# microsoft/DCVC

Hardware: AMD Instinct MI355X
Metric: 1080p YUV420 intra encode+decode pictures per second (DCVC-UF-Intra (DMCI), real rANS bit streams, q_index in {0,16,32,48,63}; sequential loop: compress then decompress per picture) (higher is better)
Workload: dtype f16

## Files before the change

### dcvc_amd/csrc/capi_ops.hip

```cpp
#include "capi_common.h"
#include <initializer_list>
#include <memory>
#include <mutex>
#include <stdexcept>
#include "dcvc_amd_ops.h"
#include "kernels/ops.h"
#include "rans/code_length.h"

namespace {

using dcvc::half_t;

inline const half_t* H(const void* p) { return static_cast<const half_t*>(p); }
inline half_t* H(void* p) { return static_cast<half_t*>(p); }
inline hipStream_t S(void* s) { return static_cast<hipStream_t>(s); }

const half_t* zero_page()
{
    static half_t* z = nullptr;
    static std::once_flag once;
    std::call_once(once, [] {
        dcvc::hip_check(hipMalloc(&z, 4096), "hipMalloc(zero page)");
        dcvc::hip_check(hipMemset(z, 0, 4096), "hipMemset(zero page)");
    });
// ... 321 lines not shown
        d.b3 = H(b3); d.b0 = H(b0); d.b2 = H(b2); d.q = H(q); d.q2 = H(q2);
        d.y = H(y); d.ldy = ldy;
        d.pixels = pixels; d.c = c; d.ci = ci; d.shortcut = shortcut != 0;
        d.wfin = wf.half(); d.bfin = H(bfin); d.qfin = H(qfin); d.yfin = H(yfin); d.ldyfin = ldyfin; d.nfin = nfin;
        dcvc::dcb_nsplit(d, st);
    });
}

int dcvc_dcb_nsplit_dw_supported(int c, int ci, int pixels)
{
    return dcvc::dcb_nsplit_dw_supported(c, ci, pixels) ? 1 : 0;
}

int dcvc_dcb_nsplit_dw(const void* t1, int ldt, const void* wdw, int width, const void* x, int ldx, const void* w3, const void* b3,
                       const void* w0, const void* b0, const void* w2, const void* b2, const void* q, const void* q2,
                       const void* w1n, const void* b1n, void* t1n, int ldt1,
                       const void* wfin, const void* bfin, const void* qfin, void* yfin, int ldyfin, int nfin,
                       void* y, int ldy, int pixels, int c, int ci, int shortcut, void* stream)
{
    return dcvc::guarded([&] {
        dcvc::kernels_init();
        nsplit_check_shape(c, ci);
        if (!t1 || !wdw || !w3 || !w0 || !w2) throw std::invalid_argument("dcb_nsplit_dw: missing operand");
        if (!dcvc::dcb_nsplit_dw_supported(c, ci, pixels)) throw std::invalid_argument("dcb_nsplit_dw: no kernel variant with the depthwise conv inside for this block shape");
        if (wfin != nullptr && !dcvc::dcb_nsplit_fin_supported(c, ci, nfin)) throw std::invalid_argument("dcb_nsplit_dw: no kernel variant for this closing conv");
        if (static_cast<long long>(pixels) * ldt * 2 >= (1LL << 31)) throw std::invalid_argument("dcb_nsplit_dw: dc.0's output must span less than 2 GiB (32-bit byte offsets inside the launch)");
        hipStream_t st = S(stream);
        const AsyncBuf wmain(dcvc::dcb_nsplit_main_halves(c, ci) * 2, st);
        dcvc::dcb_nsplit_pack_main(H(w3), H(w0), H(w2), c, ci, wmain.half(), st);
        std::unique_ptr<AsyncBuf> wnext, wf;
        if (w1n != nullptr) {
            wnext = std::make_unique<AsyncBuf>(dcvc::dcb_nsplit_dc0_halves(c, ci) * 2, st);
            dcvc::dcb_nsplit_pack_dc0(H(w1n), c, ci, wnext->half(), st);
        }
        if (wfin != nullptr) {
            wf = std::make_unique<AsyncBuf>(dcvc::dcb_nsplit_fin_halves(c, nfin) * 2, st);
            dcvc::dcb_nsplit_pack_fin(H(wfin), c, nfin, wf->half(), st);
        }
        dcvc::DcbNsplitDesc d;
        d.t1 = H(t1); d.ldt = ldt; d.wdw = H(wdw); d.width = width; d.x = H(x); d.ldx = ldx;
        d.wmain = wmain.half();
        d.wnext = wnext ? wnext->half() : nullptr;
        d.b3 = H(b3); d.b0 = H(b0); d.b2 = H(b2); d.b1n = H(b1n); d.q = H(q); d.q2 = H(q2);
        d.t1n = H(t1n); d.ldt1 = ldt1; d.y = H(y); d.ldy = ldy;
        d.pixels = pixels; d.c = c; d.ci = ci; d.shortcut = shortcut != 0;
        if (wf) { d.wfin = wf->half(); d.bfin = H(bfin); d.qfin = H(qfin); d.yfin = H(yfin); d.ldyfin = ldyfin; d.nfin = nfin; }
        dcvc::dcb_nsplit(d, st);
// ... 443 lines not shown
```

### dcvc_amd/csrc/kernels/dcb_nsplit.hip

```cpp
#include "dcb_nsplit8_kernel.h"

namespace dcvc {

using namespace nsplit;

namespace {

struct Share {
    int hi, lo, act;
    bool by_pair;
    __host__ __device__ explicit Share(int n)
    {
        by_pair = n % 128 == 0;
        if (by_pair) {
            const int q = n / 128;
            hi = (q + 1) / 2; lo = q / 2; act = 4;
        } else {
            const int tn = n / 32;
            hi = (tn + 7) / 8;
            const int rem = tn - 4 * hi;
            lo = rem <= 0 ? 0 : (rem + 3) / 4;
            act = lo == 0 ? 0 : rem / lo;
        }
    }
// ... 84 lines not shown
           (c == 512 && ci == 256) || (c == 256 && ci == 128) ||
           (c == 384 && ci == 192) ||
           (c == 192 && ci == 192);
}

bool dcb_nsplit_fin_supported(int c, int ci, int nn)
{
    static const bool off = [] { const char* e = getenv("DCVC_NSPLIT_FIN"); return e != nullptr && atoi(e) == 0; }();
    if (off || !dcb_nsplit_shape(c, ci)) return false;
    if (c == 256 && ci == 128) return nn == 128 || nn == 192 || nn == 256;
    if (c == 256 && ci == 256) return nn == 192;
    if (c == 512 && ci == 512) return nn == 256 || nn == 512;
    if (c == 768 && ci == 768) return nn == 768;
    if (c == 384 && ci == 192) return nn == 384;
    return false;
}

static bool nsplit_wide(int pixels, int c)
{
    static const bool narrow_all = [] { const char* e = getenv("DCVC_NSPLIT_PX"); return e != nullptr && atoi(e) == 32; }();
    return pixels >= 64 * 200 && c < 768 && !narrow_all;
}

bool dcb_nsplit_dw_supported(int c, int ci, int pixels)
{
    static const bool off = [] { const char* e = getenv("DCVC_NSPLIT_DW"); return e != nullptr && atoi(e) == 0; }();
    if (off || pixels <= 0) return false;
    return (c == 256 && ci == 128) || (c == 384 && ci == 192 && !nsplit_wide(pixels, c));
}

void dcb_nsplit_dw_hook(const half_t* t1, const half_t* wdw, int width)
{
    g_dw_hook_t1 = t1; g_dw_hook_taps = wdw; g_dw_hook_width = width;
}

void dcb_nsplit_timeline_buffer(long long* device_buffer)
{
    g_ns_timeline = device_buffer;
}

size_t dcb_nsplit_main_halves(int c, int ci)
{
    const Share sc(c);
    return (2ull * 4 * (sc.hi + sc.lo) * (ci / 16) + 1ull * (ci / 8) * (c / 16)) * 512;
}
size_t dcb_nsplit_dc0_halves(int c, int ci)
{
    return ci % 128 == 0 ? 1ull * (ci / 32) * (c / 16) * 512 : dcb_nsplit_fin_halves(c, ci);
}

size_t dcb_nsplit_fin_halves(int c, int nn)
// ... 33 lines not shown
}

int dcb_nsplit_waves()
{
    return 8;
}

int dcb_nsplit_mode()
{
    static const int mode = [] { const char* e = getenv("DCVC_NSPLIT"); return e != nullptr ? atoi(e) : 2; }();
    return mode;
}

bool dcb_nsplit_supported(int c, int cdc, int cffn)
{
    static const bool core_off = [] { const char* e = getenv("DCVC_NO_DCB_CORE"); return e != nullptr && atoi(e) != 0; }();
    if (core_off || dcb_nsplit_mode() == 0 || cdc != cffn || !dcb_nsplit_shape(c, cdc)) return false;
    return cdc == c || dcb_nsplit_mode() >= 2;
}

void dcb_nsplit(const DcbNsplitDesc& desc, hipStream_t stream)
{
    DcbNsplitDesc d = desc;
    if (g_dw_hook_t1 != nullptr && d.t1 == nullptr && dcb_nsplit_dw_supported(d.c, d.ci, d.pixels) && d.pixels % g_dw_hook_width == 0) {
        d.t2 = nullptr; d.t1 = g_dw_hook_t1; d.wdw = g_dw_hook_taps; d.width = g_dw_hook_width;
    }
    if (!dcb_nsplit_shape(d.c, d.ci)) {
        throw std::invalid_argument("dcb_nsplit: (block width, inner width) must be (256, 256), (384, 384), (512, 512), (768, 768), (512, 256), (256, 128), (384, 192) or (192, 192)");
    }
    if (d.pixels <= 0) throw std::invalid_argument("dcb_nsplit: empty problem");
    if ((d.ldt % 8) || (d.ldx % 8) || (d.ldy % 8) || (d.wnext && d.ldt1 % 8)) {
        throw std::invalid_argument("dcb_nsplit: leading dimensions must be multiples of 8 channels");
    }
    if (d.t1 != nullptr) {
        if (d.t2 != nullptr) throw std::invalid_argument("dcb_nsplit: either the depthwise conv's output (t2) or its input (t1)");
        if (!dcb_nsplit_dw_supported(d.c, d.ci, d.pixels)) throw std::invalid_argument("dcb_nsplit: no kernel with the depthwise conv inside for this block shape and size");
        if (!d.wdw || d.width <= 0 || d.pixels % d.width != 0) throw std::invalid_argument("dcb_nsplit: depthwise conv inside needs its taps and the picture's width");
        if (d.t1 == d.t1n) throw std::invalid_argument("dcb_nsplit: dc.0's output for the next block must not overwrite this block's (neighbouring workgroups read it)");
    }
    if ((!d.t2 && !d.t1) || !d.x || !d.wmain || !d.b3 || !d.b0 || !d.b2 || (!d.y && !d.wfin) || (d.wnext && (!d.b1n || !d.t1n))) {
        throw std::invalid_argument("dcb_nsplit: missing operand");
    }
    if (d.wfin != nullptr) {
        if (d.wnext != nullptr) throw std::invalid_argument("dcb_nsplit: a block either hands dc.0 to the next block or closes the chain");
        if (!dcb_nsplit_fin_supported(d.c, d.ci, d.nfin)) throw std::invalid_argument("dcb_nsplit: no kernel for this closing conv");
        if (!d.bfin || !d.yfin || d.ldyfin % 8) throw std::invalid_argument("dcb_nsplit: closing conv needs bias, output and a leading dimension in units of 8");
    }
    NsParams p{};
    p.t2 = d.t2; p.ldt = d.ldt; p.x = d.x; p.ldx = d.ldx;
    p.t1 = d.t1; p.wdw = d.wdw; p.W = d.width;
    p.wmain = reinterpret_cast<const half8*>(d.wmain); p.wnext = reinterpret_cast<const half8*>(d.wnext);
    p.b3 = d.b3; p.b0 = d.b0; p.b2 = d.b2; p.b1n = d.b1n; p.q = d.q; p.q2 = d.q2;
    p.wsilu = wsilu_table_device();
    p.y = d.y; p.ldy = d.ldy; p.t1n = d.t1n; p.ldt1 = d.ldt1; p.M = d.pixels; p.shortcut = d.shortcut ? 1 : 0;
    p.timeline = g_ns_timeline;
    if (d.wfin != nullptr) {
        p.wnext = reinterpret_cast<const half8*>(d.wfin); p.b1n = d.bfin; p.qf = d.qfin; p.t1n = d.yfin; p.ldt1 = d.ldyfin;
    }
    const bool wide = nsplit_wide(d.pixels, d.c);
    const int next = d.wfin != nullptr ? d.nfin : d.wnext != nullptr ? 1 : 0;
    if (d.t1 != nullptr && d.c == 384) nsplit8::run_384_192_dw(p, next, stream);
    else if (d.t1 != nullptr) nsplit8::run_256_128_dw(p, wide, next, stream);
    else if (d.c == 192) nsplit8::run_192_192(p, wide, next, stream);
    else if (d.c == 384 && d.ci == 192) nsplit8::run_384_192(p, wide, next, stream);
    else if (d.c == 384) nsplit8::run_384_384(p, wide, next, stream);
    else if (d.c == 768) nsplit8::run_768_768(p, wide, next, stream);
    else if (d.c == 512 && d.ci == 512) nsplit8::run_512_512(p, wide, next, stream);
    else if (d.c == 512) nsplit8::run_512_256(p, wide, next, stream);
    else if (d.ci == 256) nsplit8::run_256_256(p, wide, next, stream);
    else nsplit8::run_256_128(p, wide, next, stream);
}

}
```

### dcvc_amd/csrc/kernels/dcb_nsplit8_kernel.h

```cpp
#pragma once
#include "dcb_nsplit_common.h"

namespace dcvc {
namespace nsplit8 {

using nsplit::align16k;
using nsplit::lds_dma16;
using nsplit::NsParams;
using nsplit::R;
using nsplit::static_for;
using nsplit::TABLE_BYTES;
using nsplit::uint4v;

constexpr int NTHREADS = 512;
#ifndef NS8_RING
#define NS8_RING 8
#endif
constexpr int RING = NS8_RING;
#ifndef NS8_RING1
#define NS8_RING1 8
#endif
#ifndef NS8_AHEAD
#define NS8_AHEAD 2
#endif
#ifndef NS8_AHEAD_WIDE
#define NS8_AHEAD_WIDE 1
#endif
#ifndef NS8_GATHERS
#define NS8_GATHERS 8
#endif
constexpr int GB = NS8_GATHERS;

#ifndef NS8_TRIPLE
#define NS8_TRIPLE 1
#endif
template <int C, int CI, int PXT, int NEXT = 1, int DW = 0>
struct Lay {
    static constexpr int CIP = (CI + 127) / 128 * 128;
    static constexpr int CP = (C + 127) / 128 * 128;
    static constexpr int BUF_A = 32 * PXT * CIP * 2, BUF_B = 32 * PXT * CP * 2;
    static constexpr int NB = NEXT > 1 ? NEXT : CI;
    static constexpr int BIAS_FLOATS = 2 * C + 4 * CI + NB;
    static constexpr int CONSTS = BIAS_FLOATS * 4 + 2 * C * 2;
    static constexpr bool FIT4 = 2 * BUF_A + BUF_B + 4 * TABLE_BYTES + CONSTS <= 160 * 1024 && (2 * BUF_A + BUF_B) % 16384 == 0;
    static constexpr bool FIT1 = 2 * BUF_A + BUF_B + 1 * TABLE_BYTES + CONSTS <= 160 * 1024 && (2 * BUF_A + BUF_B) % 4096 == 0;
    static constexpr bool TRIPLE = NS8_TRIPLE != 0 && (FIT4 || FIT1);
    static constexpr int RT = TRIPLE ? (FIT4 ? 4 : 1) : R;
    static constexpr int OFF_B = BUF_A;
    static constexpr int OFF_A2 = BUF_A + BUF_B;
    static constexpr int OFF_TABLE = TRIPLE ? 2 * BUF_A + BUF_B : align16k(BUF_A + BUF_B);
    static constexpr int OFF_BIAS = OFF_TABLE + RT * TABLE_BYTES;
    static constexpr int OFF_Q = OFF_BIAS + BIAS_FLOATS * 4;
    static constexpr int run_chunks(int nw)
    {
        const int pxw = 32 * PXT / nw, pcs = ((pxw + 2) * (CI / 8) + 63) / 64;
        return (nw - 1) * pxw * (CI / 8) + pcs * 64;
    }
    static constexpr int rows_per_run()
    {
        const int ch = run_chunks(8) > run_chunks(4) ? run_chunks(8) : run_chunks(4);
        const int r = (ch + CI / 8 - 1) / (CI / 8);
        return r > 32 * PXT + 2 ? r : 32 * PXT + 2;
    }
    static constexpr int RH = rows_per_run();
    static constexpr int OFF_WDW = OFF_Q + 2 * C * 2;
    static constexpr int OFF_ZERO = OFF_WDW + 9 * CI * 2;
    static constexpr int OFF_H = (OFF_ZERO + 16 + 1023) & ~1023;
    static constexpr int BYTES = DW != 0 ? OFF_H + 3 * RH * CI * 2 : OFF_Q + 2 * C * 2;
    static_assert(BYTES <= 160 * 1024, "LDS budget");
    static_assert(DW == 0 || TRIPLE, "depthwise conv inside: needs the second t2 buffer");
};

template <int C, int CI>
struct Geo {
    static constexpr int KS_C = C / 16, KS_I = CI / 16;
    static constexpr int QC = C / 128, QI = CI / 128;
    static constexpr int HI_C = (QC + 1) / 2, LO_C = QC / 2;
    static constexpr int HI_I = (QI + 1) / 2, LO_I = QI / 2;
    static constexpr bool I_BY_PAIR = CI % 128 == 0;
    static constexpr int PAIRS = CI / 16, P0_HI = (PAIRS + 7) / 8, P0_LO = (PAIRS - 4 * P0_HI) / 4;
    static constexpr int TP = 2;
    static constexpr int n0(bool hiw) { return 2 * (hiw ? P0_HI : P0_LO); }
    static constexpr int np(bool hiw) { return hiw ? P0_HI : P0_LO; }
    static constexpr bool C_BY_PAIR = C % 128 == 0;
    static constexpr bool EVEN = HI_C == LO_C && HI_I == LO_I && I_BY_PAIR && C_BY_PAIR && P0_HI == P0_LO;
    static constexpr int nt_c(bool hiw) { return C_BY_PAIR ? (hiw ? HI_C : LO_C) : (nt_f(C, hiw) > 0 ? nt_f(C, hiw) : 0); }
    static constexpr int nt_i(bool hiw) { return I_BY_PAIR ? (hiw ? HI_I : LO_I) : nt_f(CI, hiw); }
    static constexpr int f_dc3(bool hiw) { return nt_c(hiw) * KS_I; }
    static constexpr int f_ffn0(bool hiw) { return n0(hiw) * KS_C; }
    static constexpr int f_main(bool hiw) { return 2 * f_dc3(hiw) + f_ffn0(hiw); }
    static constexpr int f_dc0(bool hiw) { return nt_i(hiw) * KS_C; }
// ... 8 lines not shown
    static_assert(C % 64 == 0 && CI % 64 == 0 && 4 * (P0_HI + P0_LO) == PAIRS && P0_LO >= 1, "channel counts the eight waves can share");
};

template <int C, int CI, int PXT, int NEXT, int DW, bool HIW>
__device__ __forceinline__ void block_body(const NsParams& p, char* const smem)
{
    using G = Geo<C, CI>;
    constexpr int RING = PXT == 1 ? NS8_RING1 : NS8_RING;
    constexpr bool FIN = NEXT > 1;
    static_assert(!FIN || G::fin_ok(NEXT), "closing conv: a width the eight waves can share");
    static_assert(G::I_BY_PAIR || G::fin_ok(CI), "dc.0: an inner width the eight waves can share");
    static_assert(G::C_BY_PAIR || G::fin_ok(C), "a block width the eight waves can share");
    constexpr int PX = 32 * PXT;
    constexpr int KS_C = G::KS_C, KS_I = G::KS_I;
    constexpr int NT_C = G::nt_c(HIW), NP = G::np(HIW), TP = G::TP;
    constexpr int F_DC3 = G::f_dc3(HIW), F_FFN0 = G::f_ffn0(HIW), F_MAIN = G::f_main(HIW), F_DC0 = G::f_next(NEXT, HIW);
    constexpr int NT_N = G::nt_next(NEXT, HIW);
    constexpr int CIP = Lay<C, CI, PXT, NEXT, DW>::CIP;
    constexpr int CP = Lay<C, CI, PXT, NEXT, DW>::CP;
    constexpr int CH_C = CP / 8, CH_I = CIP / 8;
    constexpr int PITCH_C = CP * 2, PITCH_I = CIP * 2;
    using L = Lay<C, CI, PXT, NEXT, DW>;
    constexpr bool TRIPLE = L::TRIPLE;
    constexpr int RT = L::RT;
    constexpr int OFF_B = L::OFF_B, OFF_A2 = L::OFF_A2;
    constexpr int OFF_TABLE = L::OFF_TABLE;
    constexpr int OFF_BIAS = L::OFF_BIAS;
    constexpr int BIAS_FLOATS = L::BIAS_FLOATS;
    constexpr int OFF_Q = L::OFF_Q;
    constexpr int TOTAL = F_MAIN + (NEXT ? F_DC0 : 0);
    static_assert((PX * CH_C) % NTHREADS == 0 && (PX * CH_I) % NTHREADS == 0, "tile rows must split evenly over the threads");

    const int tid = threadIdx.x;
    const int lane = tid & 63;
    const int wave = __builtin_amdgcn_readfirstlane(tid >> 6);
    const int simd = wave & 3;
    const int px = lane & 31;
    const int hi = lane >> 5;
    const int ntiles = (p.M + PX - 1) / PX;
    const bool banded = DW != 0 && (gridDim.x & 7) == 0 && ntiles >= static_cast<int>(gridDim.x);
    const int band0 = banded ? static_cast<int>((blockIdx.x & 7) * ntiles) >> 3 : 0;
    const int band_n = banded ? (static_cast<int>(((blockIdx.x & 7) + 1) * ntiles) >> 3) - band0 : 0;
    int slot = blockIdx.x >> 3;
    int tile = banded ? band0 + slot : static_cast<int>(blockIdx.x);
    bool first_tile = true;
    int m0 = tile * PX;
// ... 1 lines not shown
    if ((lds_base & 16383u) != 0) __builtin_trap();
    const bool upper = wave >= 4;
    const int cb_c = G::C_BY_PAIR ? 32 * (simd * G::QC + (upper ? G::HI_C : 0))
                   : HIW ? 32 * wave * G::nf_hi(C) : 32 * (4 * G::nf_hi(C) + (wave - 4) * G::nf_lo(C));
    const bool c_on = G::C_BY_PAIR || HIW || (wave - 4) < G::act_lo(C);
    const int cb_x = c_on ? cb_c : 0;
    const int cb_0 = HIW ? wave * (32 * G::n0(true)) : 4 * 32 * G::n0(true) + (wave - 4) * (32 * G::n0(false));
    constexpr bool BY_PAIR = !FIN && G::I_BY_PAIR;
    constexpr int NN = FIN ? NEXT : CI;
    const int cb_n = BY_PAIR ? 32 * (simd * G::QI + (upper ? G::HI_I : 0))
                   : HIW ? 32 * wave * G::nf_hi(NN) : 32 * (4 * G::nf_hi(NN) + (wave - 4) * G::nf_lo(NN));
    const bool nx_on = BY_PAIR || HIW || (wave - 4) < G::act_lo(NN);
    const long long rt0 = static_cast<long long>(__builtin_amdgcn_s_memrealtime());
    int stamp_no = 0;
    auto stamp = [&]() {
        if (p.timeline != nullptr && tid == 0 && stamp_no < 29 && first_tile) {
            p.timeline[static_cast<size_t>(blockIdx.x) * 32 + stamp_no] = static_cast<long long>(__builtin_readcyclecounter());
        }
        ++stamp_no;
    };
    stamp();

    static_assert(RT == 4 || RT == 1, "table slots per thread, spelled out");
    const float4 tab0 = p.wsilu[min(tid / RT, WSILU_SEGMENTS - 1)], tab1 = p.wsilu[min((tid + NTHREADS) / RT, WSILU_SEGMENTS - 1)];
    constexpr int CONST_UNITS = (BIAS_FLOATS + 2 * C) / 8;
    constexpr int CONST_PER_THREAD = (CONST_UNITS + NTHREADS - 1) / NTHREADS;
    static_assert(CONST_PER_THREAD <= 2, "two named registers below");
    auto const_unit = [&](int k) {
        const int ch = min(tid + k * NTHREADS, CONST_UNITS - 1) * 8;
        const half_t* src = ch < C ? p.b3 + ch
                          : ch < C + 4 * CI ? p.b0 + (ch - C)
                          : ch < 2 * C + 4 * CI ? p.b2 + (ch - C - 4 * CI)
                          : ch < BIAS_FLOATS ? (p.b1n != nullptr ? p.b1n + (ch - 2 * C - 4 * CI) : p.b2)
                          : ch < BIAS_FLOATS + C ? (p.q != nullptr ? p.q + (ch - BIAS_FLOATS) : p.b2)
                          : (p.q2 != nullptr ? p.q2 + (ch - BIAS_FLOATS - C) : p.b2);
        return *reinterpret_cast<const half8*>(src);
    };
    const half8 cv0 = const_unit(0), cv1 = const_unit(CONST_PER_THREAD > 1 ? 1 : 0);
    static_assert(DW == 0 || 9 * CI / 8 <= NTHREADS, "the depthwise taps: one 16-byte unit per thread");
    half8 wdv = {0, 0, 0, 0, 0, 0, 0, 0};
    if constexpr (DW != 0) wdv = *reinterpret_cast<const half8*>(p.wdw + min(tid, 9 * CI / 8 - 1) * 8);
    const float* const lb3 = reinterpret_cast<const float*>(smem + OFF_BIAS);
    const float* const lb0 = lb3 + C;
    const float* const lb2 = lb3 + C + 4 * CI;
    const float* const lb1n = lb3 + 2 * C + 4 * CI;
    const half_t* const lq = reinterpret_cast<const half_t*>(smem + OFF_Q);
    const half_t* const lq2 = lq + C;
    unsigned tab = lds_base + OFF_TABLE + (lane & (RT - 1)) * 16;

    constexpr int FM_HI = G::f_main(true), FM_LO = G::f_main(false), FD_HI = G::f_next(NEXT, true), FD_LO = G::f_next(NEXT, false);
    unsigned wsm = static_cast<unsigned>((HIW ? wave * FM_HI : 4 * FM_HI + (wave - 4) * FM_LO) * 64 + lane) * 16u;
    unsigned wsn = static_cast<unsigned>((HIW ? wave * FD_HI : nx_on ? 4 * FD_HI + (wave - 4) * FD_LO : 0) * 64 + lane) * 16u;
    const __amdgpu_buffer_rsrc_t rs_main = __builtin_amdgcn_make_buffer_rsrc(const_cast<half8*>(p.wmain), 0, 0x7fffffff, 0x00020000);
    const __amdgpu_buffer_rsrc_t rs_next = __builtin_amdgcn_make_buffer_rsrc(const_cast<half8*>(NEXT != 0 ? p.wnext : p.wmain), 0, 0x7fffffff, 0x00020000);
    half8 ring[RING];
    auto issue = [&](auto f_tag) {
        constexpr int f = decltype(f_tag)::value;
        if constexpr (f < F_MAIN) {
            ring[f % RING] = __builtin_bit_cast(half8, __builtin_amdgcn_raw_buffer_load_b128(rs_main, wsm + static_cast<unsigned>(f & 3) * 1024u, (f >> 2) * 4096, 0));
        } else if constexpr (f < TOTAL) {
            constexpr int g = f - F_MAIN;
            ring[f % RING] = __builtin_bit_cast(half8, __builtin_amdgcn_raw_buffer_load_b128(rs_next, wsn + static_cast<unsigned>(g & 3) * 1024u, (g >> 2) * 4096, 0));
        }
    };
// ... 87 lines not shown
        for (int i = 0; i < STEPS; ++i) {
            if (i + 1 < STEPS) taps(i + 1, v[(i + 1) & 1]);
            __builtin_amdgcn_sched_barrier(0);
            const int n = i * 64 + (tidv & 63);
            const int r = wi * PXW + n / CH_H, pc = n % CH_H;
            if constexpr (!FIXED_CHUNK) {
#pragma unroll
                for (int k = 0; k < 9; ++k) wt[k] = *reinterpret_cast<const half8*>(smem + L::OFF_WDW + (k * CI + pc * 8) * 2);
            }
            float acc[8];
#pragma unroll
            for (int e = 0; e < 8; ++e) acc[e] = 0.f;
#pragma unroll
            for (int k = 0; k < 9; ++k)
#pragma unroll
                for (int e = 0; e < 8; ++e) acc[e] = fmaf(static_cast<float>(v[i & 1][k][e]), static_cast<float>(wt[k][e]), acc[e]);
            half8 o;
#pragma unroll
            for (int e = 0; e < 8; ++e) o[e] = to_half(acc[e]);
            if (ITEMS % 64 == 0 || n < ITEMS) *reinterpret_cast<half8*>(smem + dst + r * PITCH_I + ((pc ^ (r & 15)) << 4)) = o;
            __builtin_amdgcn_sched_barrier(0);
        }
    };
    constexpr bool DW_ALL = G::even(NEXT);
    half8 xr[NT_C > 0 ? NT_C : 1][PXT][2];
    int pxv = px, hiv = hi;
    auto load_x = [&](int first_row) {
#pragma unroll
        for (int t = 0; t < PXT; ++t) {
            const half_t* const row = p.x + static_cast<size_t>(min(first_row + 32 * t + pxv, p.M - 1)) * p.ldx + (cb_x + 8 * hiv);
#pragma unroll
            for (int j = 0; j < NT_C; ++j)
#pragma unroll
                for (int pr = 0; pr < 2; ++pr) xr[j][t][pr] = *reinterpret_cast<const half8*>(row + 32 * j + 16 * pr);
        }
    };
    if constexpr (DW != 0) dma_halo(std::integral_constant<int, 8>{}, wave, m0);
    else dma_tile(ChI{}, p.t2, p.ldt, 0, m0);
    __builtin_amdgcn_sched_barrier(0);
    static_for<0, RING>([&](auto i) { issue(i); });
    __builtin_amdgcn_sched_barrier(0);
    load_x(m0);
    __builtin_amdgcn_sched_barrier(0);
    asm volatile("s_waitcnt vmcnt(%0)" ::"n"((DW != 0 ? H_PER_WAVE8 : PX * CH_I / NTHREADS) + RING + NT_C * PXT * 2) : "memory");
    {
        float4* t = reinterpret_cast<float4*>(smem + OFF_TABLE);
        if (RT == 4 || tid < WSILU_SEGMENTS) t[tid] = tab0;
        if (RT == 4) t[tid + NTHREADS] = tab1;
        float* lb = reinterpret_cast<float*>(smem + OFF_BIAS);
        half_t* lqw = reinterpret_cast<half_t*>(smem + OFF_Q);
        auto put = [&](int k, const half8 v) {
            const int u = tid + k * NTHREADS;
            if (u < BIAS_FLOATS / 8) {
                float4v lo4, hi4;
#pragma unroll
                for (int e = 0; e < 4; ++e) {
                    lo4[e] = static_cast<float>(v[e]);
                    hi4[e] = static_cast<float>(v[4 + e]);
                }
                *reinterpret_cast<float4v*>(lb + u * 8) = lo4;
                *reinterpret_cast<float4v*>(lb + u * 8 + 4) = hi4;
            } else if (u < CONST_UNITS) {
                *reinterpret_cast<half8*>(lqw + (u - BIAS_FLOATS / 8) * 8) = v;
            }
        };
        put(0, cv0);
        if (CONST_PER_THREAD > 1) put(1, cv1);
        if constexpr (DW != 0) {
            if (tid < 9 * CI / 8) *reinterpret_cast<half8*>(smem + L::OFF_WDW + tid * 16) = wdv;
            if (tid == NTHREADS - 1) *reinterpret_cast<half8*>(smem + L::OFF_ZERO) = half8{0, 0, 0, 0, 0, 0, 0, 0};
        }
    }
    asm volatile("s_waitcnt vmcnt(%0)" ::"n"(NT_C * PXT * 2) : "memory");
    __syncthreads();
    if constexpr (DW != 0) {
        dw_tile(std::integral_constant<int, 8>{}, wave, 0, m0);
        __syncthreads();
    }
    stamp();

    int s0 = (hi ^ (px & 15)) << 4;
    int rowA = px * PITCH_I, rowB = px * PITCH_C + OFF_B;
    int abuf = 0;
    int hi4 = 4 * hi;
    int fa8[8], fb8[8];
    auto frag_a = [&](int t, int ks) { return *reinterpret_cast<const half8*>(smem + fa8[ks & 7] + (t * (32 * PITCH_I) + (ks >> 3) * 256)); };
    auto frag_b = [&](int t, int ks) { return *reinterpret_cast<const half8*>(smem + fb8[ks & 7] + (t * (32 * PITCH_C) + (ks >> 3) * 256)); };
    auto run_a = [&](int t, int ch0) { return reinterpret_cast<half8*>(smem + rowA + t * (32 * PITCH_I) + ((ch0 * 2) ^ s0)); };
    auto run_b = [&](int t, int ch0) { return reinterpret_cast<half8*>(smem + rowB + t * (32 * PITCH_C) + ((ch0 * 2) ^ s0)); };
    auto bias_tile = [&](float16v& acc, const float* bias, int first) {
        const float* bp = bias + first + hi4;
#pragma unroll
        for (int g4 = 0; g4 < 4; ++g4) {
            const float4v b4 = *reinterpret_cast<const float4v*>(bp + 8 * g4);
#pragma unroll
            for (int e = 0; e < 4; ++e) acc[4 * g4 + e] = b4[e];
        }
    };
// ... 49 lines not shown
    const int next_tile = banded ? band0 + next_slot : tile + static_cast<int>(gridDim.x);
    const bool has_next = banded ? next_slot < band_n : next_tile < ntiles;
    if constexpr (NT_C > 0) {
        float16v acc[NT_C][PXT];
#pragma unroll
        for (int j = 0; j < NT_C; ++j)
#pragma unroll
            for (int t = 0; t < PXT; ++t) bias_tile(acc[j][t], lb3, cb_c + 32 * j);
        contract(std::integral_constant<int, NT_C>{}, KsI{}, std::integral_constant<int, 0>{}, frag_a, acc);
#pragma unroll
        for (int j = 0; j < NT_C; ++j)
#pragma unroll
            for (int t = 0; t < PXT; ++t)
#pragma unroll
                for (int pr = 0; pr < 2; ++pr) {
                    float v[8];
                    runs_of(acc[j][t], pr, v);
                    half8 o;
#pragma unroll
                    for (int e = 0; e < 8; ++e) o[e] = to_half(v[e] + static_cast<float>(xr[j][t][pr][e]));
                    *run_b(t, cb_c + 32 * j + 16 * pr) = o;
                }
    }
    __syncthreads();
    stamp();

    {
        float16v acc[TP][PXT];
        static_for<0, NP>([&](auto pass_tag) {
            constexpr int pass = decltype(pass_tag)::value;
            const int f0 = cb_0 + pass * (32 * TP);
#pragma unroll
            for (int j = 0; j < TP; ++j)
#pragma unroll
                for (int t = 0; t < PXT; ++t) bias_tile(acc[j][t], lb0, f0 + 32 * j);
            contract(std::integral_constant<int, TP>{}, KsC{}, std::integral_constant<int, F_DC3 + pass * TP * KS_C>{}, frag_b, acc);
            if constexpr (TRIPLE && pass == NP - 1) {
                if constexpr (DW != 0) {
                    if (has_next) {
                        if constexpr (DW_ALL) dma_halo(std::integral_constant<int, 8>{}, wave, next_tile * PX);
                        else if constexpr (!HIW) dma_halo(std::integral_constant<int, 4>{}, wave - 4, next_tile * PX);
                    }
                } else {
                    if (has_next) dma_tile(ChI{}, p.t2, p.ldt, abuf == 0 ? OFF_A2 : 0, next_tile * PX);
                }
                if constexpr (NT_C > 0) load_x(next_tile * PX);
                __builtin_amdgcn_sched_barrier(0);
            }
#pragma unroll
            for (int t = 0; t < PXT; ++t) {
                float sums[2][4];
#pragma unroll
                for (int h = 0; h < 2; ++h) {
#pragma unroll
                    for (int g0 = 0; g0 < 16; g0 += GB) {
                        float4v c[GB];
#pragma unroll
                        for (int e = 0; e < GB; ++e) {
                            const float4 r = wsilu_row_lds<RT, true>(acc[h][t][g0 + e], tab);
                            c[e] = float4v{r.x, r.y, r.z, r.w};
                        }
#pragma unroll
                        for (int g = 0; g < GB / 4; ++g) {
                            auto row = [&](int e) { const float4v r = c[4 * g + e]; return make_float4(r[0], r[1], r[2], r[3]); };
                            const int v0 = g0 + 4 * g;
                            float s = acc[h][t][v0] * wsilu_poly(acc[h][t][v0], row(0));
// ... 50 lines not shown
                    if (p.shortcut) {
                        const int m = min(m0 + 32 * t + px, p.M - 1);
                        const half8 r8 = *reinterpret_cast<const half8*>(p.x + static_cast<size_t>(m) * p.ldx + (cb_x + 32 * j + 16 * pr) + 8 * hi);
#pragma unroll
                        for (int e = 0; e < 8; ++e) v[e] = v[e] + static_cast<float>(r8[e]);
                    }
                    if (p.q != nullptr) {
                        const half8 q8 = *reinterpret_cast<const half8*>(lq + ch + 8 * hi);
#pragma unroll
                        for (int e = 0; e < 8; ++e) v[e] = v[e] * static_cast<float>(q8[e]);
                    }
                    half8 o;
#pragma unroll
                    for (int e = 0; e < 8; ++e) o[e] = to_half(v[e]);
                    if (p.q2 != nullptr) {
                        const half8 q8 = *reinterpret_cast<const half8*>(lq2 + ch + 8 * hi);
#pragma unroll
                        for (int e = 0; e < 8; ++e) o[e] = hmul(o[e], q8[e]);
                    }
                    if constexpr (NEXT != 0) *slot = o;
                    const int m = m0 + 32 * t + pxv;
                    if (m < p.M && c_on && (!FIN || p.y != nullptr)) store_line(p.y + static_cast<size_t>(m) * p.ldy + ch + 8 * hiv, o);
                }
    }
    if constexpr (NEXT != 0) __syncthreads();
    stamp();
    if constexpr (NEXT != 0 && NT_N > 0) {
        if (nx_on) {
            float16v acc[NT_N][PXT];
#pragma unroll
            for (int j = 0; j < NT_N; ++j)
#pragma unroll
                for (int t = 0; t < PXT; ++t) bias_tile(acc[j][t], lb1n, cb_n + 32 * j);
            contract(std::integral_constant<int, NT_N>{}, KsC{}, std::integral_constant<int, F_MAIN>{}, frag_b, acc);
            if (has_next) {
                __builtin_amdgcn_sched_barrier(0);
                static_for<0, RING>([&](auto i) { issue(i); });
                __builtin_amdgcn_sched_barrier(0);
            }
            stamp();
#pragma unroll
            for (int j = 0; j < NT_N; ++j)
#pragma unroll
                for (int t = 0; t < PXT; ++t)
#pragma unroll
                    for (int pr = 0; pr < 2; ++pr) {
// ... 17 lines not shown
                            }
#pragma unroll
                            for (int e = 0; e < 8; ++e) o[e] = to_half(v[e]);
                        }
                        const int m = m0 + 32 * t + pxv;
                        if (m < p.M) store_line(p.t1n + static_cast<size_t>(m) * p.ldt1 + cb_n + 32 * j + 16 * pr + 8 * hiv, o);
                    }
        } else {
            if (has_next) {
                __builtin_amdgcn_sched_barrier(0);
                static_for<0, RING>([&](auto i) { issue(i); });
                __builtin_amdgcn_sched_barrier(0);
            }
            stamp();
        }
    } else {
        if (has_next) {
            __builtin_amdgcn_sched_barrier(0);
            static_for<0, RING>([&](auto i) { issue(i); });
            __builtin_amdgcn_sched_barrier(0);
        }
        stamp();
    }
    if constexpr (DW != 0) {
        if (has_next) {
            if constexpr (DW_ALL || !HIW) asm volatile("s_waitcnt vmcnt(%0)" ::"n"(RING) : "memory");
            if constexpr (DW_ALL) dw_tile(std::integral_constant<int, 8>{}, wave, abuf == 0 ? OFF_A2 : 0, next_tile * PX);
            else if constexpr (!HIW) dw_tile(std::integral_constant<int, 4>{}, wave - 4, abuf == 0 ? OFF_A2 : 0, next_tile * PX);
        }
    }
    stamp();
    if (!has_next) break;
    asm volatile("s_waitcnt vmcnt(0)" ::: "memory");
    __syncthreads();
    stamp();
    tile = next_tile;
    slot = next_slot;
    first_tile = false;
    m0 = tile * PX;
    if constexpr (TRIPLE) {
        abuf = abuf == 0 ? OFF_A2 : 0;
        rowA = pxv * PITCH_I + abuf;
    }
    }
    if (p.timeline != nullptr && tid == 0) {
        p.timeline[static_cast<size_t>(blockIdx.x) * 32 + 31] = static_cast<long long>(__builtin_readcyclecounter());
        p.timeline[static_cast<size_t>(blockIdx.x) * 32 + 30] = static_cast<long long>(__builtin_amdgcn_s_memrealtime());
// ... 68 lines not shown
}

template <int C, int CI, int PXT, int... FINS>
void run_px8_dw(const NsParams& p, int next, hipStream_t stream)
{
    if (next == 0) { launch8<C, CI, PXT, 0, 1>(p, stream); return; }
    if (next == 1) { launch8<C, CI, PXT, 1, 1>(p, stream); return; }
    const bool hit = ((next == FINS ? (launch8<C, CI, PXT, FINS, 1>(p, stream), true) : false) || ... || false);
    if (!hit) throw std::invalid_argument("dcb_nsplit8: no instantiation for a closing conv of width " + std::to_string(next));
}

template <int C, int CI, int... FINS>
void run_shape8(const NsParams& p, bool wide, int next, hipStream_t stream)
{
    if constexpr (C < 768) {
        if (wide) { run_px8<C, CI, 2, FINS...>(p, next, stream); return; }
    }
    run_px8<C, CI, 1, FINS...>(p, next, stream);
}

void run_256_128(const NsParams& p, bool wide, int next, hipStream_t stream);
void run_256_128_dw(const NsParams& p, bool wide, int next, hipStream_t stream);
void run_384_192_dw(const NsParams& p, int next, hipStream_t stream);
void run_256_256(const NsParams& p, bool wide, int next, hipStream_t stream);
void run_192_192(const NsParams& p, bool wide, int next, hipStream_t stream);
void run_384_192(const NsParams& p, bool wide, int next, hipStream_t stream);
void run_384_384(const NsParams& p, bool wide, int next, hipStream_t stream);
void run_512_256(const NsParams& p, bool wide, int next, hipStream_t stream);
void run_512_512(const NsParams& p, bool wide, int next, hipStream_t stream);
void run_768_768(const NsParams& p, bool wide, int next, hipStream_t stream);

}
}
```

### dcvc_amd/csrc/kernels/ops.h

```cpp
#pragma once

#include <hip/hip_runtime.h>

#include <cstdint>
#include <stdexcept>
#include <string>

namespace dcvc {

typedef _Float16 half_t;

inline void hip_check(hipError_t e, const char* what)
{
    if (e != hipSuccess) {
        throw std::runtime_error(std::string(what) + ": " + hipGetErrorString(e));
    }
}

void kernels_init();

void gemm_profile_enable(bool on);
void gemm_profile_reset();
void gemm_profile_collect(double* ms, double* flops, long long* launches);
struct GemmLaunchInfo {
// ... 13 lines not shown
    const half_t* q = nullptr;
    const half_t* q2 = nullptr;
    half_t* y = nullptr; int ldy = 0;
    int pixels = 0, cin = 0, cout = 0;
    bool wsilu = false, chunk_add = false;
};
void conv1x1(const Conv1x1Desc& d, hipStream_t stream);

struct DcbNsplitDesc {
    const half_t* t2 = nullptr; int ldt = 0;
    const half_t* x = nullptr; int ldx = 0;
    const half_t* wmain = nullptr;
    const half_t* wnext = nullptr;
    const half_t* b3 = nullptr; const half_t* b0 = nullptr; const half_t* b2 = nullptr; const half_t* b1n = nullptr;
    const half_t* q = nullptr; const half_t* q2 = nullptr;
    half_t* t1n = nullptr; int ldt1 = 0;
    half_t* y = nullptr; int ldy = 0;
    int pixels = 0, c = 0, ci = 0;
    bool shortcut = false;
    const half_t* wfin = nullptr; const half_t* bfin = nullptr; const half_t* qfin = nullptr;
    half_t* yfin = nullptr; int ldyfin = 0; int nfin = 0;
    const half_t* t1 = nullptr; const half_t* wdw = nullptr; int width = 0;
};
bool dcb_nsplit_dw_supported(int c, int ci, int pixels);
int dcb_nsplit_waves();
bool dcb_nsplit_shape(int c, int ci);
bool dcb_nsplit_supported(int c, int cdc, int cffn);
size_t dcb_nsplit_main_halves(int c, int ci);
size_t dcb_nsplit_dc0_halves(int c, int ci);
void dcb_nsplit_pack_main(const half_t* w3, const half_t* w0, const half_t* w2, int c, int ci, half_t* out, hipStream_t stream);
void dcb_nsplit_pack_dc0(const half_t* w1, int c, int ci, half_t* out, hipStream_t stream);
bool dcb_nsplit_fin_supported(int c, int ci, int nn);
size_t dcb_nsplit_fin_halves(int c, int nn);
void dcb_nsplit_pack_fin(const half_t* w , int c, int nn, half_t* out, hipStream_t stream);
void dcb_nsplit(const DcbNsplitDesc& d, hipStream_t stream);
void dcb_nsplit_timeline_buffer(long long* device_buffer);
void dcb_nsplit_dw_hook(const half_t* t1, const half_t* wdw, int width);

struct DcbPairDesc {
    const half_t* x = nullptr; int ldx = 0;
    const half_t* wa = nullptr; const half_t* ba = nullptr;
    const half_t* w1 = nullptr; const half_t* b1 = nullptr;
    half_t* y = nullptr; int ldy = 0;
    half_t* t1 = nullptr; int ldt1 = 0;
    int pixels = 0, cin = 0, c = 0, ci = 0;
};
// ... 251 lines not shown
```

Measured before the change: 147.5.

## Add register-based depthwise conv variant of fused nsplit block for 384x384

```diff
diff --git a/dcvc_amd/csrc/capi_ops.hip b/dcvc_amd/csrc/capi_ops.hip
--- a/dcvc_amd/csrc/capi_ops.hip
+++ b/dcvc_amd/csrc/capi_ops.hip
@@ -367,7 +367,7 @@
         dcvc::kernels_init();
         nsplit_check_shape(c, ci);
         if (!t1 || !wdw || !w3 || !w0 || !w2) throw std::invalid_argument("dcb_nsplit_dw: missing operand");
-        if (!dcvc::dcb_nsplit_dw_supported(c, ci, pixels)) throw std::invalid_argument("dcb_nsplit_dw: no kernel variant with the depthwise conv inside for this block shape");
+        if (!dcvc::dcb_nsplit_dw_available(c, ci, pixels)) throw std::invalid_argument("dcb_nsplit_dw: no kernel variant with the depthwise conv inside for this block shape");
         if (wfin != nullptr && !dcvc::dcb_nsplit_fin_supported(c, ci, nfin)) throw std::invalid_argument("dcb_nsplit_dw: no kernel variant for this closing conv");
         if (static_cast<long long>(pixels) * ldt * 2 >= (1LL << 31)) throw std::invalid_argument("dcb_nsplit_dw: dc.0's output must span less than 2 GiB (32-bit byte offsets inside the launch)");
         hipStream_t st = S(stream);
diff --git a/dcvc_amd/csrc/kernels/dcb_nsplit.hip b/dcvc_amd/csrc/kernels/dcb_nsplit.hip
--- a/dcvc_amd/csrc/kernels/dcb_nsplit.hip
+++ b/dcvc_amd/csrc/kernels/dcb_nsplit.hip
@@ -130,11 +130,16 @@
     return pixels >= 64 * 200 && c < 768 && !narrow_all;
 }
 
-bool dcb_nsplit_dw_supported(int c, int ci, int pixels)
+bool dcb_nsplit_dw_available(int c, int ci, int pixels)
 {
     static const bool off = [] { const char* e = getenv("DCVC_NSPLIT_DW"); return e != nullptr && atoi(e) == 0; }();
     if (off || pixels <= 0) return false;
-    return (c == 256 && ci == 128) || (c == 384 && ci == 192 && !nsplit_wide(pixels, c));
+    return (c == 256 && ci == 128) || (c == 384 && ci == 192 && !nsplit_wide(pixels, c)) || (c == 384 && ci == 384 && nsplit_wide(pixels, c));
+}
+
+bool dcb_nsplit_dw_supported(int c, int ci, int pixels)
+{
+    return dcb_nsplit_dw_available(c, ci, pixels) && !(c == 384 && ci == 384);
 }
 
 void dcb_nsplit_dw_hook(const half_t* t1, const half_t* wdw, int width)
@@ -214,7 +219,7 @@
 void dcb_nsplit(const DcbNsplitDesc& desc, hipStream_t stream)
 {
     DcbNsplitDesc d = desc;
-    if (g_dw_hook_t1 != nullptr && d.t1 == nullptr && dcb_nsplit_dw_supported(d.c, d.ci, d.pixels) && d.pixels % g_dw_hook_width == 0) {
+    if (g_dw_hook_t1 != nullptr && d.t1 == nullptr && dcb_nsplit_dw_available(d.c, d.ci, d.pixels) && d.pixels % g_dw_hook_width == 0) {
         d.t2 = nullptr; d.t1 = g_dw_hook_t1; d.wdw = g_dw_hook_taps; d.width = g_dw_hook_width;
     }
     if (!dcb_nsplit_shape(d.c, d.ci)) {
@@ -226,8 +231,9 @@
     }
     if (d.t1 != nullptr) {
         if (d.t2 != nullptr) throw std::invalid_argument("dcb_nsplit: either the depthwise conv's output (t2) or its input (t1)");
-        if (!dcb_nsplit_dw_supported(d.c, d.ci, d.pixels)) throw std::invalid_argument("dcb_nsplit: no kernel with the depthwise conv inside for this block shape and size");
+        if (!dcb_nsplit_dw_available(d.c, d.ci, d.pixels)) throw std::invalid_argument("dcb_nsplit: no kernel with the depthwise conv inside for this block shape and size");
         if (!d.wdw || d.width <= 0 || d.pixels % d.width != 0) throw std::invalid_argument("dcb_nsplit: depthwise conv inside needs its taps and the picture's width");
+        if (static_cast<long long>(d.pixels) * d.ldt * 2 >= (1LL << 31)) throw std::invalid_argument("dcb_nsplit: dc.0's output must span less than 2 GiB (32-bit byte offsets inside the launch)");
         if (d.t1 == d.t1n) throw std::invalid_argument("dcb_nsplit: dc.0's output for the next block must not overwrite this block's (neighbouring workgroups read it)");
     }
     if ((!d.t2 && !d.t1) || !d.x || !d.wmain || !d.b3 || !d.b0 || !d.b2 || (!d.y && !d.wfin) || (d.wnext && (!d.b1n || !d.t1n))) {
@@ -251,7 +257,8 @@
     }
     const bool wide = nsplit_wide(d.pixels, d.c);
     const int next = d.wfin != nullptr ? d.nfin : d.wnext != nullptr ? 1 : 0;
-    if (d.t1 != nullptr && d.c == 384) nsplit8::run_384_192_dw(p, next, stream);
+    if (d.t1 != nullptr && d.c == 384 && d.ci == 384) nsplit8::run_384_384_dw(p, next, stream);
+    else if (d.t1 != nullptr && d.c == 384) nsplit8::run_384_192_dw(p, next, stream);
     else if (d.t1 != nullptr) nsplit8::run_256_128_dw(p, wide, next, stream);
     else if (d.c == 192) nsplit8::run_192_192(p, wide, next, stream);
     else if (d.c == 384 && d.ci == 192) nsplit8::run_384_192(p, wide, next, stream);
diff --git a/dcvc_amd/csrc/kernels/dcb_nsplit8_kernel.h b/dcvc_amd/csrc/kernels/dcb_nsplit8_kernel.h
--- a/dcvc_amd/csrc/kernels/dcb_nsplit8_kernel.h
+++ b/dcvc_amd/csrc/kernels/dcb_nsplit8_kernel.h
@@ -28,6 +28,9 @@
 #endif
 #ifndef NS8_GATHERS
 #define NS8_GATHERS 8
+#endif
+#ifndef NS8_DW_AHEAD
+#define NS8_DW_AHEAD (1 | 1 << 2 | 1 << 4 | 1 << 6)
 #endif
 constexpr int GB = NS8_GATHERS;
 
@@ -66,7 +69,8 @@
     static constexpr int OFF_WDW = OFF_Q + 2 * C * 2;
     static constexpr int OFF_ZERO = OFF_WDW + 9 * CI * 2;
     static constexpr int OFF_H = (OFF_ZERO + 16 + 1023) & ~1023;
-    static constexpr int BYTES = DW != 0 ? OFF_H + 3 * RH * CI * 2 : OFF_Q + 2 * C * 2;
+    static constexpr bool DW_REG = DW != 0 && OFF_H + 3 * RH * CI * 2 > 160 * 1024;
+    static constexpr int BYTES = DW != 0 && !DW_REG ? OFF_H + 3 * RH * CI * 2 : OFF_Q + 2 * C * 2;
     static_assert(BYTES <= 160 * 1024, "LDS budget");
     static_assert(DW == 0 || TRIPLE, "depthwise conv inside: needs the second t2 buffer");
 };
@@ -121,6 +125,9 @@
     constexpr int PITCH_C = CP * 2, PITCH_I = CIP * 2;
     using L = Lay<C, CI, PXT, NEXT, DW>;
     constexpr bool TRIPLE = L::TRIPLE;
+    constexpr bool DW_REG = L::DW_REG;
+    constexpr bool DW_LDS = DW != 0 && !DW_REG;
+    static_assert(!DW_REG || (CI % 64 == 0 && PX % 16 == 0 && !Geo<C, CI>::even(NEXT)), "dw_reg: lines of 8 chunks, 8 pixels per wave step, the waves 4 .. 7 with the smaller share");
     constexpr int RT = L::RT;
     constexpr int OFF_B = L::OFF_B, OFF_A2 = L::OFF_A2;
     constexpr int OFF_TABLE = L::OFF_TABLE;
@@ -168,6 +175,7 @@
     stamp();
 
     static_assert(RT == 4 || RT == 1, "table slots per thread, spelled out");
+    constexpr int REG_Q8 = (CI / 64) * (PX / 8) / 8, REG_Q4 = (CI / 64) * (PX / 8) / 4;
     const float4 tab0 = p.wsilu[min(tid / RT, WSILU_SEGMENTS - 1)], tab1 = p.wsilu[min((tid + NTHREADS) / RT, WSILU_SEGMENTS - 1)];
     constexpr int CONST_UNITS = (BIAS_FLOATS + 2 * C) / 8;
     constexpr int CONST_PER_THREAD = (CONST_UNITS + NTHREADS - 1) / NTHREADS;
@@ -183,9 +191,9 @@
         return *reinterpret_cast<const half8*>(src);
     };
     const half8 cv0 = const_unit(0), cv1 = const_unit(CONST_PER_THREAD > 1 ? 1 : 0);
-    static_assert(DW == 0 || 9 * CI / 8 <= NTHREADS, "the depthwise taps: one 16-byte unit per thread");
+    static_assert(!DW_LDS || 9 * CI / 8 <= NTHREADS, "the depthwise taps: one 16-byte unit per thread");
     half8 wdv = {0, 0, 0, 0, 0, 0, 0, 0};
-    if constexpr (DW != 0) wdv = *reinterpret_cast<const half8*>(p.wdw + min(tid, 9 * CI / 8 - 1) * 8);
+    if constexpr (DW_LDS) wdv = *reinterpret_cast<const half8*>(p.wdw + min(tid, 9 * CI / 8 - 1) * 8);
     const float* const lb3 = reinterpret_cast<const float*>(smem + OFF_BIAS);
     const float* const lb0 = lb3 + C;
     const float* const lb2 = lb3 + C + 4 * CI;
@@ -319,6 +327,120 @@
             __builtin_amdgcn_sched_barrier(0);
         }
     };
+    auto dw_reg = [&](auto n_tag, auto same_tag, auto piece_tag, int q0, int dst, int first_row) {
+        constexpr int N = decltype(n_tag)::value;
+        constexpr bool SAME_GROUP = decltype(same_tag)::value;
+        constexpr int BLK = PX / 8;
+        const int fr = __builtin_amdgcn_readfirstlane(first_row);
+        const int qs = __builtin_amdgcn_readfirstlane(q0);
+        int W = p.W, row_b = p.ldt * 2;
+        asm volatile("" : "+s"(W), "+s"(row_b));
+        const int y0 = fr / W, x0 = fr - y0 * W;
+        const int lp = (tidv & 63) >> 3, lc = tidv & 7;
+        unsigned lane_off[3];
+#pragma unroll
+        for (int kx = 0; kx < 3; ++kx) lane_off[kx] = static_cast<unsigned>((lp + kx) * row_b + lc * 16);
+        const __amdgpu_buffer_rsrc_t rs_t1 = __builtin_amdgcn_make_buffer_rsrc(const_cast<half_t*>(p.t1), 0, 0x7fffffff, 0x00020000);
+        const __amdgpu_buffer_rsrc_t rs_wdw = __builtin_amdgcn_make_buffer_rsrc(const_cast<half_t*>(p.wdw), 0, 9 * CI * 2, 0x00020000);
+        half8 wt[9];
+        auto load_taps = [&](int g) {
+#pragma unroll
+            for (int k = 0; k < 9; ++k) wt[k] = __builtin_bit_cast(half8, __builtin_amdgcn_raw_buffer_load_b128(rs_wdw, static_cast<unsigned>(lc * 16), (k * CI + g * 64) * 2, 0));
+        };
+        struct Pos { int g, r_lo, xf, yf; bool inner; };
+        auto pos = [&](int q) {
+            Pos s;
+            s.g = q / BLK; s.r_lo = (q % BLK) * 8;
+            s.xf = x0 + s.r_lo; s.yf = y0;
+            while (s.xf >= W) { s.xf -= W; ++s.yf; }
+            s.inner = s.yf > 0 && fr + s.r_lo + 7 + W < p.M && s.xf >= 1 && s.xf + 8 < W;
+            return s;
+        };
+        struct Ops { half8 c[3], e[3]; };
+        const bool first_px = lp == 0, last_px = lp == 7;
+        auto taps = [&](int q, Ops& o) {
+            const Pos s = pos(q);
+            const int m_lo = fr + s.r_lo;
+#pragma unroll
+            for (int ky = 0; ky < 3; ++ky) o.e[ky] = half8{0, 0, 0, 0, 0, 0, 0, 0};
+            if (s.inner) {
+#pragma unroll
+                for (int ky = 0; ky < 3; ++ky) {
+                    const int so = (m_lo - 1 + (ky - 1) * W) * row_b + s.g * 128;
+                    o.c[ky] = __builtin_bit_cast(half8, __builtin_amdgcn_raw_buffer_load_b128(rs_t1, lane_off[1], so, 0));
+                    if (first_px || last_px) {
+                        o.e[ky] = __builtin_bit_cast(half8, __builtin_amdgcn_raw_buffer_load_b128(rs_t1, first_px ? lane_off[0] : lane_off[2], so, 0));
+                    }
+                }
+            } else {
+                const int m = m_lo + lp;
+#pragma unroll
+                for (int ky = 0; ky < 3; ++ky) {
+                    const int src = min(max(m + (ky - 1) * W, 0), p.M - 1);
+                    o.c[ky] = __builtin_bit_cast(half8, __builtin_amdgcn_raw_buffer_load_b128(rs_t1, static_cast<unsigned>(src * row_b + lc * 16), s.g * 128, 0));
+                    if (first_px || last_px) {
+                        const int se = min(max(m + (ky - 1) * W + (first_px ? -1 : 1), 0), p.M - 1);
+                        o.e[ky] = __builtin_bit_cast(half8, __builtin_amdgcn_raw_buffer_load_b128(rs_t1, static_cast<unsigned>(se * row_b + lc * 16), s.g * 128, 0));
+                    }
+                }
+            }
+        };
+        const int lane_lo = (((tidv & 63) - 8) & 63) * 4, lane_hi = (((tidv & 63) + 8) & 63) * 4;
+        load_taps(qs / BLK);
+        constexpr int AH = (NS8_DW_AHEAD >> (2 * decltype(piece_tag)::value)) & 3;
+        Ops ops[AH + 1];
+#pragma unroll
+        for (int i = 0; i < AH && i < N; ++i) taps(qs + i, ops[i]);
+#pragma unroll
+        for (int i = 0; i < N; ++i) {
+            const int q = qs + i;
+            if (i + AH < N || AH == 0) taps(q + AH, ops[(i + AH) % (AH + 1)]);
+            __builtin_amdgcn_sched_barrier(0);
+            const Ops& o = ops[i % (AH + 1)];
+            const Pos s = pos(q);
+            const int r = s.r_lo + lp, pc = s.g * 8 + lc;
+            int xx = s.xf + lp, yy = s.yf;
+            if (!s.inner) {
+                while (xx >= W) { xx -= W; ++yy; }
+            }
+            const bool up = s.inner || yy > 0, down = s.inner || fr + r + W < p.M, left = s.inner || xx > 0, right = s.inner || xx + 1 < W;
+            float acc[8];
+#pragma unroll
+            for (int e = 0; e < 8; ++e) acc[e] = 0.f;
+#pragma unroll
+            for (int ky = 0; ky < 3; ++ky) {
+                const uint4v cc = __builtin_bit_cast(uint4v, o.c[ky]), ee = __builtin_bit_cast(uint4v, o.e[ky]);
+                uint4v vl, vr;
+#pragma unroll
+                for (int d = 0; d < 4; ++d) {
+                    const unsigned a = static_cast<unsigned>(__builtin_amdgcn_ds_bpermute(lane_lo, static_cast<int>(cc[d])));
+                    const unsigned b = static_cast<unsigned>(__builtin_amdgcn_ds_bpermute(lane_hi, static_cast<int>(cc[d])));
+                    vl[d] = first_px ? ee[d] : a;
+                    vr[d] = last_px ? ee[d] : b;
+                }
+                const bool row_ok = (ky != 0 || up) && (ky != 2 || down);
+                const half8 zero = {0, 0, 0, 0, 0, 0, 0, 0};
+                const half8 v3[3] = {row_ok && left ? __builtin_bit_cast(half8, vl) : zero, row_ok ? o.c[ky] : zero,
+                                     row_ok && right ? __builtin_bit_cast(half8, vr) : zero};
+#pragma unroll
+                for (int kx = 0; kx < 3; ++kx)
+#pragma unroll
+                    for (int e = 0; e < 8; ++e) acc[e] = fmaf(static_cast<float>(v3[kx][e]), static_cast<float>(wt[3 * ky + kx][e]), acc[e]);
+            }
+            half8 ov;
+#pragma unroll
+            for (int e = 0; e < 8; ++e) ov[e] = to_half(acc[e]);
+            *reinterpret_cast<half8*>(smem + dst + r * PITCH_I + ((pc ^ (r & 15)) << 4)) = ov;
+            if constexpr (!SAME_GROUP) {
+                if (i + 1 < N && (q + 1) % BLK == 0) load_taps((q + 1) / BLK);
+            }
+            __builtin_amdgcn_sched_barrier(0);
+        }
+    };
+    constexpr int REG_WIN = 3;
+    static_assert(!DW_REG || ((CI / 64) * (PX / 8) % 8 == 0 && REG_Q4 % REG_WIN == 0), "dw_reg: whole steps per wave and piece");
+    using RegSteps = std::integral_constant<int, DW_REG ? REG_Q4 / REG_WIN : 1>;
+    using RegSame = std::bool_constant<(PX / 8) % RegSteps::value == 0>;
     constexpr bool DW_ALL = G::even(NEXT);
     half8 xr[NT_C > 0 ? NT_C : 1][PXT][2];
     int pxv = px, hiv = hi;
@@ -332,14 +454,14 @@
                 for (int pr = 0; pr < 2; ++pr) xr[j][t][pr] = *reinterpret_cast<const half8*>(row + 32 * j + 16 * pr);
         }
     };
-    if constexpr (DW != 0) dma_halo(std::integral_constant<int, 8>{}, wave, m0);
-    else dma_tile(ChI{}, p.t2, p.ldt, 0, m0);
+    if constexpr (DW_LDS) dma_halo(std::integral_constant<int, 8>{}, wave, m0);
+    else if constexpr (DW == 0) dma_tile(ChI{}, p.t2, p.ldt, 0, m0);
     __builtin_amdgcn_sched_barrier(0);
     static_for<0, RING>([&](auto i) { issue(i); });
     __builtin_amdgcn_sched_barrier(0);
     load_x(m0);
     __builtin_amdgcn_sched_barrier(0);
-    asm volatile("s_waitcnt vmcnt(%0)" ::"n"((DW != 0 ? H_PER_WAVE8 : PX * CH_I / NTHREADS) + RING + NT_C * PXT * 2) : "memory");
+    asm volatile("s_waitcnt vmcnt(%0)" ::"n"((DW_REG ? 0 : DW != 0 ? H_PER_WAVE8 : PX * CH_I / NTHREADS) + RING + NT_C * PXT * 2) : "memory");
     {
         float4* t = reinterpret_cast<float4*>(smem + OFF_TABLE);
         if (RT == 4 || tid < WSILU_SEGMENTS) t[tid] = tab0;
@@ -363,14 +485,19 @@
         };
         put(0, cv0);
         if (CONST_PER_THREAD > 1) put(1, cv1);
-        if constexpr (DW != 0) {
+        if constexpr (DW_LDS) {
             if (tid < 9 * CI / 8) *reinterpret_cast<half8*>(smem + L::OFF_WDW + tid * 16) = wdv;
             if (tid == NTHREADS - 1) *reinterpret_cast<half8*>(smem + L::OFF_ZERO) = half8{0, 0, 0, 0, 0, 0, 0, 0};
         }
     }
-    asm volatile("s_waitcnt vmcnt(%0)" ::"n"(NT_C * PXT * 2) : "memory");
-    __syncthreads();
-    if constexpr (DW != 0) {
+    if constexpr (!DW_REG) {
+        asm volatile("s_waitcnt vmcnt(%0)" ::"n"(NT_C * PXT * 2) : "memory");
+        __syncthreads();
+    }
+    if constexpr (DW_REG) {
+        dw_reg(std::integral_constant<int, REG_Q8>{}, std::false_type{}, std::integral_constant<int, 0>{}, wave * REG_Q8, 0, m0);
+        __syncthreads();
+    } else if constexpr (DW != 0) {
         dw_tile(std::integral_constant<int, 8>{}, wave, 0, m0);
         __syncthreads();
     }
@@ -466,6 +593,9 @@
                     *run_b(t, cb_c + 32 * j + 16 * pr) = o;
                 }
     }
+    if constexpr (DW_REG && !HIW) {
+        if (has_next) dw_reg(RegSteps{}, RegSame{}, std::integral_constant<int, 1>{}, (wave - 4) * REG_Q4, abuf == 0 ? OFF_A2 : 0, next_tile * PX);
+    }
     __syncthreads();
     stamp();
 
@@ -480,12 +610,12 @@
                 for (int t = 0; t < PXT; ++t) bias_tile(acc[j][t], lb0, f0 + 32 * j);
             contract(std::integral_constant<int, TP>{}, KsC{}, std::integral_constant<int, F_DC3 + pass * TP * KS_C>{}, frag_b, acc);
             if constexpr (TRIPLE && pass == NP - 1) {
-                if constexpr (DW != 0) {
+                if constexpr (DW_LDS) {
                     if (has_next) {
                         if constexpr (DW_ALL) dma_halo(std::integral_constant<int, 8>{}, wave, next_tile * PX);
                         else if constexpr (!HIW) dma_halo(std::integral_constant<int, 4>{}, wave - 4, next_tile * PX);
                     }
-                } else {
+                } else if constexpr (DW == 0) {
                     if (has_next) dma_tile(ChI{}, p.t2, p.ldt, abuf == 0 ? OFF_A2 : 0, next_tile * PX);
                 }
                 if constexpr (NT_C > 0) load_x(next_tile * PX);
@@ -582,6 +712,9 @@
                     const int m = m0 + 32 * t + pxv;
                     if (m < p.M && c_on && (!FIN || p.y != nullptr)) store_line(p.y + static_cast<size_t>(m) * p.ldy + ch + 8 * hiv, o);
                 }
+    }
+    if constexpr (DW_REG && !HIW) {
+        if (has_next) dw_reg(RegSteps{}, RegSame{}, std::integral_constant<int, 2>{}, (wave - 4) * REG_Q4 + RegSteps::value, abuf == 0 ? OFF_A2 : 0, next_tile * PX);
     }
     if constexpr (NEXT != 0) __syncthreads();
     stamp();
@@ -645,7 +778,10 @@
         }
         stamp();
     }
-    if constexpr (DW != 0) {
+    if constexpr (DW_REG && !HIW) {
+        if (has_next) dw_reg(RegSteps{}, RegSame{}, std::integral_constant<int, 3>{}, (wave - 4) * REG_Q4 + 2 * RegSteps::value, abuf == 0 ? OFF_A2 : 0, next_tile * PX);
+    }
+    if constexpr (DW_LDS) {
         if (has_next) {
             if constexpr (DW_ALL || !HIW) asm volatile("s_waitcnt vmcnt(%0)" ::"n"(RING) : "memory");
             if constexpr (DW_ALL) dw_tile(std::integral_constant<int, 8>{}, wave, abuf == 0 ? OFF_A2 : 0, next_tile * PX);
@@ -760,6 +896,7 @@
 void run_256_128(const NsParams& p, bool wide, int next, hipStream_t stream);
 void run_256_128_dw(const NsParams& p, bool wide, int next, hipStream_t stream);
 void run_384_192_dw(const NsParams& p, int next, hipStream_t stream);
+void run_384_384_dw(const NsParams& p, int next, hipStream_t stream);
 void run_256_256(const NsParams& p, bool wide, int next, hipStream_t stream);
 void run_192_192(const NsParams& p, bool wide, int next, hipStream_t stream);
 void run_384_192(const NsParams& p, bool wide, int next, hipStream_t stream);
diff --git a/dcvc_amd/csrc/kernels/dcb_nsplit_dwreg_384_384.hip b/dcvc_amd/csrc/kernels/dcb_nsplit_dwreg_384_384.hip
--- /dev/null
+++ b/dcvc_amd/csrc/kernels/dcb_nsplit_dwreg_384_384.hip
@@ -0,0 +1,12 @@
+#include "dcb_nsplit8_kernel.h"
+
+namespace dcvc {
+namespace nsplit8 {
+
+void run_384_384_dw(const NsParams& p, int next, hipStream_t stream)
+{
+    run_px8_dw<384, 384, 2>(p, next, stream);
+}
+
+}
+}
diff --git a/dcvc_amd/csrc/kernels/ops.h b/dcvc_amd/csrc/kernels/ops.h
--- a/dcvc_amd/csrc/kernels/ops.h
+++ b/dcvc_amd/csrc/kernels/ops.h
@@ -59,6 +59,7 @@
     half_t* yfin = nullptr; int ldyfin = 0; int nfin = 0;
     const half_t* t1 = nullptr; const half_t* wdw = nullptr; int width = 0;
 };
+bool dcb_nsplit_dw_available(int c, int ci, int pixels);
 bool dcb_nsplit_dw_supported(int c, int ci, int pixels);
 int dcb_nsplit_waves();
 bool dcb_nsplit_shape(int c, int ci);
```

After: 153.1, median of 5. 1.04x the previous value.
